# dfm/george

Measured on NVIDIA H100. Metric: gp.compute+log_likelihood N-points/sec, higher is better.
Workload: dtype f64

## Files before the change

george_b200/csrc/hodlr.cu:

```cuda
#include <algorithm>
#include <cmath>
#include <cstdlib>
#include <cstring>
#include <vector>

#include "common.cuh"
#include "hodlr_kernels.cuh"
#include "hodlr_lu.cuh"
#include "hodlr_aca2.cuh"
#include "hodlr_leaf.cuh"
#include "linalg.cuh"
#include "kernel_eval.cuh"

namespace bgp {
int upload_program(const DevProgram& P, DevBuf<DevProgram>& buf, cudaStream_t s);
int kmat_grad_contract_launch(const DevProgram* dprog, int nd, int np, const unsigned* which_dev, const double* x,
                              int64_t n, const double* M, int64_t ldm, const double* alpha, double ca, double cm,
                              double* g_dev, double* diag_dev, DevBuf<double>& scratch, cudaStream_t s);
int fill_identity_launch(double* A, int64_t n, cudaStream_t s);
int64_t grad_slab_partial_size(int64_t n, int64_t c, int np);
int64_t grad_slab_tile_size(int64_t n, int np);
int kmat_grad_slab_launch(const DevProgram* dprog, int nd, int np, const unsigned* which_dev, const double* x, int64_t n,
                          const double* W, int64_t j0, int64_t nc, int64_t jlo, int64_t jhi, const double* alpha,
                          double* partial, double* tile_part, double* diag_dev, cudaStream_t s);
// ... 10 lines not shown
                       const double* kdiag, double* var, DevBuf<double>& scratch, cudaStream_t s);
int kmat_x1_grad_matvec_launch(const DevProgram& P, const DevProgram* dprog, const double* x1, int64_t n1,
                               const double* x2, int64_t n2, const double* V, int64_t ldv, double scale, int add_prior,
                               double* out, DevBuf<double>& scratch, cudaStream_t s);
void predict_gemm_plan(int64_t m, int64_t nn, int64_t K, int64_t* nsplit_out, int64_t* klen_out);
int predict_gemm_sub(const double* A, int64_t lda, const double* B, int64_t ldb, int64_t m, int64_t nn, int64_t K,
                     bool lower, double* C, int64_t ldc, DevBuf<double>& slices, DevBuf<GemmDesc>& descs, cudaStream_t s);
bool comm_ready();
int comm_rank();
int comm_world();
int comm_allreduce_sum_f64(double* buf, size_t count, cudaStream_t s);
int comm_allgather_f64(const double* send, double* recv, size_t count, cudaStream_t s);
}
using namespace bgp;

struct HNode {
  int start, size, half, is_leaf, parent, dir, depth;
  int slot;
  int rank = 0, draws = 0, fallback = 0;
  int owned = 1;
  int top = 0;
};

struct PanelSet {
  DevBuf<double> V, U;
  int64_t ld = 0, row_off = 0;
  int vcols = 0, ucols = 0;
  double* vbase() const { return V.p - row_off; }
  double* ubase() const { return U.p - row_off; }
};

struct LevelInfo {
  std::vector<int> nodes;
  int set = 1;
  int cap = 0, max_cap = 0, vcol = 0, r = 0, ucol = 0;
  int max_half = 0, grow = 0;
  int desc_off = 0;
};

struct AcaGraphKey {
  A2Args a;
  int nn, ncc, nrc, shape, grid;
};

struct bgp_hodlr {
  cudaStream_t sA = nullptr, sB = nullptr;
  cudaEvent_t ev[8] = {nullptr};
  int64_t n = 0;
  int ndim = 0;
  bgp_hodlr_opts_t opts;
  bool computed = false;
  double log_det = 0.0;
  DevProgram prog;

  std::vector<HNode> nodes;
  std::vector<int> leaves;
  std::vector<LevelInfo> levels;
  std::vector<int> piv_off;
  std::vector<int> h_piv_rows, h_piv_cols;
  int max_leaf = 0, rtot = 0, vcols = 0, cut_depth = 0;
  int64_t row0 = 0, nloc = 0;
  std::vector<int64_t> shard_row0, shard_rows;
  bool top_pending = false;

  DevBuf<DevProgram> d_prog;
  DevBuf<double> d_x, d_yerr, d_diag, d_L, d_leaf_logdet, d_node_logdet, d_S, d_W, d_scalar, d_rhs;
  PanelSet top, loc;
  const PanelSet& pset(const LevelInfo& L) const { return L.set == 0 ? top : loc; }
  DevBuf<double> d_inv, d_gscratch;
  DevBuf<double> d_xsend, d_xrecv;
  DevBuf<unsigned> d_which;
  LuWorkspace lu_ws;
  DevBuf<GemmDesc> d_gram_desc, d_upd_desc;
  std::vector<NodeDesc> h_nodes;
  std::vector<int> cap_hint;
  int64_t cap_hint_n = -1;
  int cap_hint_min_size = -1;
  DevBuf<LeafDesc> d_leaves;
  DevBuf<AcaDesc> d_aca;
  DevBuf<AcaOut> d_aca_out;
  DevBuf<NodeDesc> d_nodes;
  DevBuf<PanelTile> d_ptiles;
  int small_limit = SS_MAX_N;
  bool leaf_cols_wide = false;
  DevBuf<int> d_idx, d_piv_rows, d_piv_cols, d_ticket, d_chain_done, d_ncols_by_depth;
  DevBuf<uint32_t> d_chain_state;
  DevBuf<A2Node> d_a2nodes;
  DevBuf<A2State> d_a2states;
  DevBuf<MT19937> d_a2rngs;
  DevBuf<A2EPart> d_epart;
  DevBuf<int> d_cand, d_cand_k, d_cand_words, d_cand_L, d_cand_next, d_cand_live, d_cchunk_node, d_rchunk_node, d_nactive;
  DevBuf<double> d_node_box;
  DevBuf<double2> d_cand_xu, d_gbox, d_cbox;
  DevBuf<unsigned long long> d_cmax, d_stats;
  DevBuf<int4> d_work;
  DevBuf<int> d_work_count, d_iter;
  AcaGraphKey aca_key;
  cudaGraph_t aca_graph = nullptr;
  cudaGraphExec_t aca_exec = nullptr;
  cudaStream_t sC = nullptr;
  bool profile = false;
  std::vector<cudaEvent_t> prof_events;
  double prof[12] = {0, 0, 0, 0, 0, 0, 0, 0, 0, 0, 0, 0};
  uint64_t draw_paths[4] = {0, 0, 0, 0};
  uint64_t eval_units[2] = {0, 0};
  DevBuf<double> d_vpart, d_upart, d_vmax;
  int aca_iters = 0;
  size_t w_cap = 0;

  double t_ms[5] = {0, 0, 0, 0, 0};
  double grad_t[4] = {0, 0, 0, 0};
  double work[6] = {0, 0, 0, 0, 0, 0};
};

static int ensure_streams(bgp_hodlr* h) {
  if (!h->sA) {
    BGP_CUDA(cudaStreamCreateWithFlags(&h->sA, cudaStreamNonBlocking));
    BGP_CUDA(cudaStreamCreateWithFlags(&h->sB, cudaStreamNonBlocking));
    for (int i = 0; i < 8; ++i) BGP_CUDA(cudaEventCreate(&h->ev[i]));
  }
  return BGP_OK;
}

static void build_tree(bgp_hodlr* h, int start, int size, int dir, int parent, int depth) {
  HNode nd;
  nd.start = start; nd.size = size; nd.half = size / 2; nd.dir = dir; nd.parent = parent; nd.depth = depth;
  nd.is_leaf = !(nd.half >= h->opts.min_size);
  nd.slot = 0;
  const int id = (int)h->nodes.size();
  h->nodes.push_back(nd);
  if (!nd.is_leaf) {
    build_tree(h, start, nd.half, 0, id, depth + 1);
    build_tree(h, start + nd.half, size - nd.half, 1, id, depth + 1);
  }
}

static int hodlr_solve_dev(bgp_hodlr* h, double* b, int64_t nrhs, int64_t ldb, cudaStream_t s, int part,
                           int64_t eye_row0 = -1);
static int hodlr_exchange_finish(bgp_hodlr* h);

static bool host_exchange(const bgp_hodlr* h) {
  return h->opts.shard_count > 1 &&
         !(comm_ready() && comm_world() == h->opts.shard_count && comm_rank() == h->opts.shard_rank);
}

static int reject_host_exchange(const bgp_hodlr* h, const char* what) {
  if (!host_exchange(h)) return BGP_OK;
  set_error("%s is not available on a host-exchange shard (shard %d of %d without a matching communicator): use "
            "bgp_hodlr_solve_local_dev / bgp_hodlr_solve_top_dev", what, h->opts.shard_rank, h->opts.shard_count);
  return BGP_ERR_INVALID;
}
static int hodlr_finish_top_impl(bgp_hodlr* h, bool allreduce);

constexpr size_t LS_SMEM_MAX = 200 * 1024;
constexpr int LS_MAX_LEAF = (int)(LS_SMEM_MAX / sizeof(double));

static bool leaf_solve_fits(int max_leaf, int cols) { return sizeof(double) * (size_t)max_leaf * cols <= LS_SMEM_MAX; }

static void set_sweep_func_attrs() {
  static std::atomic<uint64_t> done{0};
  int dev = 0;
  cudaGetDevice(&dev);
  const uint64_t bit = dev < 64 ? (1ull << dev) : 0;
  if (bit && (done.load(std::memory_order_relaxed) & bit)) return;
  cudaFuncSetAttribute(leaf_solve_kernel<1>, cudaFuncAttributeMaxDynamicSharedMemorySize, (int)LS_SMEM_MAX);
  cudaFuncSetAttribute(leaf_solve_kernel<2>, cudaFuncAttributeMaxDynamicSharedMemorySize, (int)LS_SMEM_MAX);
  cudaFuncSetAttribute(leaf_solve_kernel<4>, cudaFuncAttributeMaxDynamicSharedMemorySize, (int)LS_SMEM_MAX);
  cudaFuncSetAttribute(leaf_solve_kernel<LS_COLS>, cudaFuncAttributeMaxDynamicSharedMemorySize, (int)LS_SMEM_MAX);
  cudaFuncSetAttribute(leaf_solve_kernel<LS_COLS_WIDE>, cudaFuncAttributeMaxDynamicSharedMemorySize, (int)LS_SMEM_MAX);
  cudaFuncSetAttribute(small_solve_kernel, cudaFuncAttributeMaxDynamicSharedMemorySize, 160 * 1024);
  done.fetch_or(bit, std::memory_order_relaxed);
}

template <int COLS>
static int leaf_solve_launch(bgp_hodlr* h, double* X, int64_t ldx, const int* ncols_by_depth, int ncols_fixed,
                             int max_cols, cudaStream_t s, int l0, int l1) {
  const int ngroups = (max_cols + COLS - 1) / COLS;
  const dim3 grid((unsigned)((size_t)(l1 - l0) * (size_t)ngroups));
  const size_t smem = sizeof(double) * (size_t)h->max_leaf * COLS;
  leaf_solve_kernel<COLS><<<grid, LS_THREADS, smem, s>>>(h->d_leaves.p + l0, h->d_L.p, X, ldx, ncols_by_depth,
                                                         ncols_fixed, h->max_leaf, ngroups);
  BGP_LAUNCH_CHECK();
  return BGP_OK;
}

static int launch_leaf_solve(bgp_hodlr* h, double* X, int64_t ldx, const int* ncols_by_depth, int ncols_fixed,
                             int max_cols, cudaStream_t s, int l0 = 0, int l1 = -1) {
  if (l1 < 0) l1 = (int)h->leaves.size();
  const int nl = l1 - l0;
  if (nl <= 0 || max_cols == 0) return BGP_OK;
  const int m = h->max_leaf;
  if (h->leaf_cols_wide && max_cols > LS_COLS && leaf_solve_fits(m, LS_COLS_WIDE))
    return leaf_solve_launch<LS_COLS_WIDE>(h, X, ldx, ncols_by_depth, ncols_fixed, max_cols, s, l0, l1);
  int cols = max_cols <= 1 ? 1 : max_cols <= 2 ? 2 : max_cols <= 4 ? 4 : LS_COLS;
  while (cols > 1 && !leaf_solve_fits(m, cols)) cols /= 2;
  if (!leaf_solve_fits(m, cols)) {
    set_error("leaf size %d too large for the leaf solve kernel (at most %d rows)", m, LS_MAX_LEAF);
    return BGP_ERR_INVALID;
  }
  switch (cols) {
    case LS_COLS: return leaf_solve_launch<LS_COLS>(h, X, ldx, ncols_by_depth, ncols_fixed, max_cols, s, l0, l1);
    case 4: return leaf_solve_launch<4>(h, X, ldx, ncols_by_depth, ncols_fixed, max_cols, s, l0, l1);
    case 2: return leaf_solve_launch<2>(h, X, ldx, ncols_by_depth, ncols_fixed, max_cols, s, l0, l1);
    default: return leaf_solve_launch<1>(h, X, ldx, ncols_by_depth, ncols_fixed, max_cols, s, l0, l1);
  }
}

static int launch_level_big(bgp_hodlr* h, const LevelInfo& L, double* X, int64_t ldx, int ncolsW, int own_off, int factor,
                            int col_lo, int col_hi, cudaStream_t s, int b0, int b1);

static int launch_level(bgp_hodlr* h, const LevelInfo& L, double* X, int64_t ldx, int ncolsW, int own_off, int factor,
                        int col_lo, int col_hi, cudaStream_t s, int b0 = 0, int b1 = -1) {
  if (b1 < 0) b1 = (int)L.nodes.size();
  const int nn = b1 - b0;
  if (nn <= 0 || L.r == 0) {
    return BGP_OK;
  }
  const int r = L.r;
  const int64_t stride = (int64_t)2 * r * ncolsW;
  const size_t need = (size_t)nn * stride;
  if (need > h->w_cap) { set_error("internal: W workspace too small (%zu > %zu)", need, h->w_cap); return BGP_ERR_CUDA; }
  BGP_CUDA(cudaMemsetAsync(h->d_W.p, 0, sizeof(double) * need, s));
  if (2 * r > h->small_limit) return launch_level_big(h, L, X, ldx, ncolsW, own_off, factor, col_lo, col_hi, s, b0, b1);
  const NodeDesc* nd = h->d_nodes.p + L.desc_off + b0;
  const int max_nh = L.max_half + 1;
  if (r <= GTS_MAX_R) {
    dim3 grid((max_nh + GTS_ROWS - 1) / GTS_ROWS, nn * 2, (ncolsW + GTS_TC - 1) / GTS_TC);
    const double* vb = h->pset(L).vbase();
    const int64_t ldv = h->pset(L).ld;
    if (r <= 2) gram_tn_small_kernel<2><<<grid, GTS_THREADS, 0, s>>>(nd, vb, ldv, X, ldx, ncolsW, h->d_W.p, stride);
    else if (r <= 4) gram_tn_small_kernel<4><<<grid, GTS_THREADS, 0, s>>>(nd, vb, ldv, X, ldx, ncolsW, h->d_W.p, stride);
    else gram_tn_small_kernel<GTS_MAX_R><<<grid, GTS_THREADS, 0, s>>>(nd, vb, ldv, X, ldx, ncolsW, h->d_W.p, stride);
    BGP_LAUNCH_CHECK();
  } else {
    dim3 grid((max_nh + GT_CHUNK - 1) / GT_CHUNK, nn * 2, (ncolsW + GT_TC - 1) / GT_TC);
    gram_tn_kernel<<<grid, GT_THREADS, 0, s>>>(nd, h->pset(L).vbase(), h->pset(L).ld, X, ldx, ncolsW, h->d_W.p, stride);
    BGP_LAUNCH_CHECK();
  }
  {
    const size_t sbytes = sizeof(double) * (size_t)(2 * r) * (2 * r);
    small_solve_kernel<<<nn, SS_THREADS, sbytes, s>>>(nd, h->d_W.p, stride, ncolsW, own_off, factor, h->d_S.p,
                                                      h->d_node_logdet.p, L.desc_off + b0);
    BGP_LAUNCH_CHECK();
  }
  if (col_hi > col_lo) {
    dim3 grid((max_nh + UP_ROWS - 1) / UP_ROWS, nn * 2, (col_hi - col_lo + UP_TC - 1) / UP_TC);
    update_nn_kernel<<<grid, UP_THREADS, 0, s>>>(nd, h->pset(L).ubase(), h->pset(L).ld, X, ldx, col_lo, col_hi, h->d_W.p, stride, 0);
    BGP_LAUNCH_CHECK();
  }
  return BGP_OK;
}

static int launch_level_big(bgp_hodlr* h, const LevelInfo& L, double* X, int64_t ldx, int ncolsW, int own_off, int factor,
                            int col_lo, int col_hi, cudaStream_t s, int b0, int b1) {
  const int nn = b1 - b0;
  const int r = L.r, n2 = 2 * r;
  const int64_t stride = (int64_t)n2 * ncolsW;
  const int64_t ldv = h->pset(L).ld, ldu = h->pset(L).ld;
  double* W = h->d_W.p;
  constexpr int KCHUNK = 4096;
  std::vector<LuNode> lun(nn);
  std::vector<GemmDesc> gram, upd;
  int max_nh = 0;
  for (int k = 0; k < nn; ++k) {
    const int b = b0 + k;
    const HNode& nd = h->nodes[L.nodes[b]];
    const int64_t s_off = h->h_nodes[L.desc_off + b].s_off;
    lun[k].S = h->d_S.p + s_off;
    lun[k].piv = reinterpret_cast<int*>(lun[k].S + (int64_t)n2 * n2);
    lun[k].logdet = h->d_node_logdet.p + L.desc_off + b;
    double* Wn = W + (int64_t)k * stride;
    for (int hh = 0; hh < 2; ++hh) {
      const int rs = nd.start + (hh ? nd.half : 0), nh = hh ? (nd.size - nd.half) : nd.half;
      max_nh = std::max(max_nh, nh);
      for (int k0 = 0; k0 < nh; k0 += KCHUNK) {
        GemmDesc g;
// ... 202 lines not shown
    BGP_CUDA(cudaMemcpyAsync(act2, h->d_nactive.p, sizeof(int) * 2, cudaMemcpyDeviceToHost, s));
    BGP_CUDA(cudaStreamSynchronize(s));
    iters = it_host;
    g_launches.fetch_add((uint64_t)7 * (uint64_t)std::max(iters - 1, 0), std::memory_order_relaxed);
    if (act2[0] > 0) { set_error("ACA did not terminate"); return BGP_ERR_CUDA; }
  } else {
    while (active > 0) {
      for (int rep = 0; rep < 8; ++rep) {
        BGP_TRY(launch_iteration(s, 0, 0, h->profile ? iters : -1));
        iters++;
      }
      int act2[2] = {0, 0};
      BGP_CUDA(cudaMemcpyAsync(act2, h->d_nactive.p, sizeof(int) * 2, cudaMemcpyDeviceToHost, s));
      BGP_CUDA(cudaStreamSynchronize(s));
      active = act2[0];
      if (iters > (1 << 22)) { set_error("ACA did not terminate"); return BGP_ERR_CUDA; }
    }
  }
  h->aca_iters = iters;
  {
    unsigned long long st4[A2_NSTATS] = {0};
    BGP_CUDA(cudaMemcpyAsync(st4, h->d_stats.p, sizeof(st4), cudaMemcpyDeviceToHost, s));
    BGP_CUDA(cudaStreamSynchronize(s));
    for (int k = 0; k < 4; ++k) h->draw_paths[k] = st4[A2_PATH_REDO + k];
    h->eval_units[0] = st4[A2_UNITS_PULLED]; h->eval_units[1] = st4[A2_UNITS_LIVE];
    h->prof[1] = iters; h->prof[2] = (double)st4[0]; h->prof[3] = (double)st4[1]; h->prof[4] = (double)st4[2];
    h->prof[5] = (double)st4[3];
    if (h->profile) {
      double tot[6] = {0, 0, 0, 0, 0, 0};
      for (int i = 0; i < iters; ++i)
        for (int k = 0; k < 6; ++k) {
          float ms = 0;
          cudaEventElapsedTime(&ms, h->prof_events[(size_t)7 * i + k], h->prof_events[(size_t)7 * i + k + 1]);
          tot[k] += ms;
        }
      h->prof[0] = tot[0];
      for (int k = 0; k < 6; ++k) h->prof[6 + k] = tot[k];
    }
  }
  if (h->opts.exhaust_mode == BGP_EXHAUST_DENSE) {
    a2_dense_fill_kernel<<<dim3(nn, 64), 256, 0, s>>>(a);
    BGP_LAUNCH_CHECK();
    a2_dense_rank_kernel<<<(nn + 127) / 128, 128, 0, s>>>(a);
    BGP_LAUNCH_CHECK();
  }
  std::vector<A2State> hs(nn);
  BGP_CUDA(cudaMemcpyAsync(hs.data(), h->d_a2states.p, sizeof(A2State) * nn, cudaMemcpyDeviceToHost, s));
  BGP_CUDA(cudaStreamSynchronize(s));
  for (int i = 0; i < nn; ++i) {
    AcaOut o;
    o.rank = hs[i].rank; o.draws = hs[i].draws; o.fallback = hs[i].fallback; o.status = hs[i].status;
    houts[descs[i].node] = o;
  }
  return BGP_OK;
}

static int hodlr_compute_dev_impl(bgp_hodlr* h, const bgp_kernel_spec_t* spec, const double* x_dev, int64_t n,
                                  int32_t ndim, const double* yerr_dev, const bgp_hodlr_opts_t* opts_in) {
  h->computed = false;
  h->top_pending = false;
  for (uint64_t& c : h->draw_paths) c = 0;
  for (uint64_t& c : h->eval_units) c = 0;
  h->shard_row0.clear(); h->shard_rows.clear();
  BGP_TRY(require_device());
  BGP_TRY(ensure_streams(h));
  BGP_TRY(build_dev_program(spec, &h->prog));
  if (h->prog.ndim != ndim) { set_error("dimension mismatch: kernel ndim %d, input ndim %d", h->prog.ndim, ndim); return BGP_ERR_DIM; }
  if (ndim > ACA_MAX_NDIM) { set_error("HODLR supports at most %d input dimensions", ACA_MAX_NDIM); return BGP_ERR_INVALID; }
  if (n <= 0 || n > (int64_t)0x7fffffff) { set_error("invalid number of points %lld", (long long)n); return BGP_ERR_INVALID; }
  bgp_hodlr_opts_t o;
  if (opts_in) o = *opts_in; else bgp_hodlr_default_opts(&o);
  if (o.min_size < 1) { set_error("min_size must be >= 1"); return BGP_ERR_INVALID; }
  if (o.shard_count < 1) o.shard_count = 1;
  if (o.shard_count & (o.shard_count - 1)) { set_error("shard_count must be a power of two"); return BGP_ERR_INVALID; }
  if (o.shard_rank < 0 || o.shard_rank >= o.shard_count) { set_error("invalid shard_rank"); return BGP_ERR_INVALID; }
  if (o.shard_count > 1 && o.rng_mode == BGP_RNG_REFERENCE) { set_error("rng_mode=reference serialises the tree and cannot be sharded"); return BGP_ERR_INVALID; }
  h->opts = o;
  h->n = n;
  h->ndim = ndim;
  cudaStream_t sA = h->sA, sB = h->sB;
  set_sweep_func_attrs();
  h->small_limit = SS_MAX_N;
  if (const char* e = getenv("BGP_SMALL_RANK_LIMIT")) h->small_limit = std::min(SS_MAX_N, atoi(e));
  h->leaf_cols_wide = false;
  if (const char* e = getenv("BGP_LEAF_COLS")) h->leaf_cols_wide = atoi(e) > LS_COLS;

  h->nodes.clear(); h->leaves.clear(); h->levels.clear();
  h->nodes.reserve(2 * (size_t)(n / std::max(1, o.min_size)) + 8);
  build_tree(h, 0, (int)n, 0, -1, 0);
  int cut = 0;
  while ((1 << cut) < o.shard_count) cut++;
  h->cut_depth = cut;
  int max_depth = 0;
  for (auto& nd : h->nodes) max_depth = std::max(max_depth, nd.depth);
  h->row0 = 0; h->nloc = n;
  if (o.shard_count > 1) {
    int seen = 0; bool found = false;
    for (size_t i = 0; i < h->nodes.size(); ++i) {
      HNode& nd = h->nodes[i];
      if (nd.depth == cut) {
        if (seen == o.shard_rank) { h->row0 = nd.start; h->nloc = nd.size; found = true; }
        h->shard_row0.push_back(nd.start); h->shard_rows.push_back(nd.size);
        seen++;
      }
    }
    if (!found || seen != o.shard_count) {
      h->shard_row0.clear(); h->shard_rows.clear();
      set_error("tree too shallow to shard %d ways (N=%lld, min_size=%d)", o.shard_count, (long long)n, o.min_size);
      return BGP_ERR_INVALID;
    }
    for (auto& nd : h->nodes) {
      nd.top = nd.depth < cut;
      nd.owned = !nd.top && nd.start >= h->row0 && nd.start + nd.size <= h->row0 + h->nloc;
    }
  }
  h->levels.assign(max_depth + 1, LevelInfo());
  for (size_t i = 0; i < h->nodes.size(); ++i) {
    HNode& nd = h->nodes[i];
    if (nd.is_leaf) { if (nd.owned) { nd.slot = (int)h->leaves.size(); h->leaves.push_back((int)i); } continue; }
    if (!(nd.owned || nd.top)) continue;
    LevelInfo& L = h->levels[nd.depth];
    nd.slot = (int)L.nodes.size();
    L.nodes.push_back((int)i);
    L.max_half = std::max(L.max_half, nd.size - nd.half);
  }
  while (!h->levels.empty() && h->levels.back().nodes.empty()) h->levels.pop_back();
  const int nlev = (int)h->levels.size();
  for (int l = 0; l < nlev; ++l) h->levels[l].set = (o.shard_count > 1 && l < cut) ? 0 : 1;
  h->top.ld = n; h->top.row_off = 0;
  h->loc.ld = h->nloc; h->loc.row_off = h->row0;

  const int rcap0 = o.rank_capacity > 0 ? o.rank_capacity : 128;
  for (auto& L : h->levels) {
    int mh = 0;
    for (int id : L.nodes) mh = std::max(mh, h->nodes[id].half);
    L.max_cap = std::max(1, mh);
    L.cap = std::min(rcap0, L.max_cap);
  }
  if (o.rank_capacity <= 0 && h->cap_hint_n == n && h->cap_hint_min_size == o.min_size && (int)h->cap_hint.size() == nlev)
    for (int l = 0; l < nlev; ++l) h->levels[l].cap = std::min(h->levels[l].max_cap, std::max(h->levels[l].cap, h->cap_hint[l]));

  BGP_TRY(upload_program(h->prog, h->d_prog, sA));
  BGP_TRY(h->d_x.reserve((size_t)n * ndim, sA));
  BGP_TRY(h->d_diag.reserve((size_t)n, sA));
  if (x_dev != h->d_x.p) BGP_CUDA(cudaMemcpyAsync(h->d_x.p, x_dev, sizeof(double) * n * ndim, cudaMemcpyDeviceToDevice, sA));
  square_kernel<<<(unsigned)std::min<int64_t>((n + 255) / 256, 1184), 256, 0, sA>>>(yerr_dev, h->d_diag.p, n);
  BGP_LAUNCH_CHECK();
  BGP_CUDA(cudaEventRecord(h->ev[0], sA));

  const int nl = (int)h->leaves.size();
  std::vector<LeafDesc> hleaves(nl);
  int64_t loff = 0;
  h->max_leaf = 0;
  for (int i = 0; i < nl; ++i) {
    const HNode& nd = h->nodes[h->leaves[i]];
    hleaves[i].start = nd.start; hleaves[i].size = nd.size; hleaves[i].depth = nd.depth; hleaves[i]._pad = 0;
    hleaves[i].off = loff;
    loff += (int64_t)nd.size * nd.size;
    h->max_leaf = std::max(h->max_leaf, nd.size);
  }
  if (h->max_leaf > LS_MAX_LEAF) {
    set_error("leaf size %d too large: the leaf solve handles at most %d rows (N=%lld, min_size=%d); lower min_size",
              h->max_leaf, LS_MAX_LEAF, (long long)n, o.min_size);
    return BGP_ERR_INVALID;
  }
  BGP_TRY(h->d_leaves.reserve(std::max(nl, 1), sA));
  BGP_TRY(h->d_L.reserve((size_t)std::max<int64_t>(loff, 1), sA));
  BGP_TRY(h->d_leaf_logdet.reserve(std::max(nl, 1), sA));
  if (nl) {
    BGP_CUDA(cudaMemcpyAsync(h->d_leaves.p, hleaves.data(), sizeof(LeafDesc) * nl, cudaMemcpyHostToDevice, sA));
    const char* lf_env = getenv("BGP_LEAF_FACTOR");
    const bool generic = lf_env && strcmp(lf_env, "generic") == 0;
    if (h->max_leaf <= LF_MAX_LEAF && !generic) {
      leaf_factor_launch(h->prog.shape, nl, h->max_leaf, sA, h->d_prog.p, h->d_x.p, h->d_diag.p, h->d_leaves.p, h->d_L.p,
                         h->d_leaf_logdet.p);
    } else {
      leaf_build_factor_kernel<<<nl, LEAF_THREADS, 0, sA>>>(h->d_prog.p, h->d_x.p, h->d_diag.p, h->d_leaves.p, h->d_L.p,
                                                            h->d_leaf_logdet.p);
    }
    BGP_LAUNCH_CHECK();
  }
  BGP_CUDA(cudaEventRecord(h->ev[1], sA));

  std::vector<AcaDesc> hdesc;
  std::vector<int> desc_node;
  std::vector<AcaOut> houts;
  int64_t idx_total = 0, piv_total = 0;
  int nint = 0;
  BGP_CUDA(cudaStreamWaitEvent(sB, h->ev[1], 0));
  for (int attempt = 0;; ++attempt) {
    int vcols_set[2] = {0, 0};
    for (auto& L : h->levels) { L.vcol = vcols_set[L.set]; vcols_set[L.set] += L.cap; }
    h->top.vcols = vcols_set[0]; h->loc.vcols = vcols_set[1];
    h->vcols = vcols_set[0] + vcols_set[1];
    hdesc.clear(); desc_node.clear();
    h->piv_off.assign(h->nodes.size(), -1);
    idx_total = 0; piv_total = 0; nint = 0;
    for (int l = 0; l < nlev; ++l) {
      for (int id : h->levels[l].nodes) {
        const HNode& nd = h->nodes[id];
        AcaDesc d;
        d.row0 = nd.start + nd.half; d.n_rows = nd.size - nd.half; d.col0 = nd.start; d.n_cols = nd.half;
        d.vcol = h->levels[l].vcol; d.cap = h->levels[l].cap; d.pre_id = id; d.node = nint;
        d.idx_off = idx_total; d.piv_off = piv_total;
        h->piv_off[id] = (int)piv_total;
        idx_total += d.n_rows; piv_total += d.cap;
        hdesc.push_back(d); desc_node.push_back(id);
        nint++;
      }
    }
    std::vector<int> order(nint);
    for (int i = 0; i < nint; ++i) order[i] = i;
    if (o.rng_mode == BGP_RNG_REFERENCE) std::sort(order.begin(), order.end(), [&](int a, int b) { return hdesc[a].pre_id < hdesc[b].pre_id; });
    else std::stable_sort(order.begin(), order.end(), [&](int a, int b) {
      const int ta = h->nodes[hdesc[a].pre_id].top, tb = h->nodes[hdesc[b].pre_id].top;
      if (ta != tb) return ta > tb;
      return hdesc[a].n_rows > hdesc[b].n_rows;
    });
    std::vector<AcaDesc> hdesc_sorted(nint);
    for (int i = 0; i < nint; ++i) hdesc_sorted[i] = hdesc[order[i]];

    {
      const size_t need_top = (size_t)n * std::max(h->top.vcols, 1), need_loc = (size_t)h->nloc * std::max(h->loc.vcols, 1);
      if ((h->top.V.p && h->top.V.n < need_top) || (h->loc.V.p && h->loc.V.n < need_loc)) {
        if (h->top.V.n < need_top) h->top.V.release();
        if (h->loc.V.n < need_loc) h->loc.V.release();
        h->top.U.release(); h->loc.U.release();
        BGP_CUDA(cudaStreamSynchronize(sA)); BGP_CUDA(cudaStreamSynchronize(sB));
        cudaMemPool_t pool; int dev = 0;
        cudaGetDevice(&dev);
        if (cudaDeviceGetDefaultMemPool(&pool, dev) == cudaSuccess) cudaMemPoolTrimTo(pool, 0);
      }
      BGP_TRY(h->top.V.reserve(need_top, sB));
      BGP_TRY(h->loc.V.reserve(need_loc, sB));
    }
    BGP_TRY(h->d_aca.reserve(std::max(nint, 1), sB));
    BGP_TRY(h->d_aca_out.reserve(std::max(nint, 1), sB));
    BGP_TRY(h->d_idx.reserve((size_t)std::max<int64_t>(idx_total, 1), sB));
    BGP_TRY(h->d_piv_rows.reserve((size_t)std::max<int64_t>(piv_total, 1), sB));
    BGP_TRY(h->d_piv_cols.reserve((size_t)std::max<int64_t>(piv_total, 1), sB));
    BGP_TRY(h->d_ticket.reserve(1, sB));
    BGP_TRY(h->d_chain_state.reserve(640, sB));
    BGP_TRY(h->d_chain_done.reserve(std::max(nint, 1), sB));
    houts.assign(nint, AcaOut());
    if (nint && o.rng_mode != BGP_RNG_REFERENCE) {
      BGP_TRY(run_aca2(h, hdesc_sorted, houts, sB));
    } else if (nint) {
      BGP_CUDA(cudaMemcpyAsync(h->d_aca.p, hdesc_sorted.data(), sizeof(AcaDesc) * nint, cudaMemcpyHostToDevice, sB));
      BGP_CUDA(cudaMemsetAsync(h->d_ticket.p, 0, sizeof(int), sB));
      BGP_CUDA(cudaMemsetAsync(h->d_chain_done.p, 0, sizeof(int) * nint, sB));
      int maxcap = 1;
      for (auto& L : h->levels) maxcap = std::max(maxcap, L.cap);
      const size_t smem = ((sizeof(AcaShared) + 15) & ~size_t(15)) + sizeof(double) * (size_t)maxcap;
      cudaFuncSetAttribute(aca_kernel, cudaFuncAttributeMaxDynamicSharedMemorySize, 200 * 1024);
      if (smem > 200 * 1024) { set_error("rank capacity %d too large", maxcap); return BGP_ERR_RANK_CAPACITY; }
      aca_kernel<<<nint, ACA_THREADS, smem, sB>>>(h->d_prog.p, h->d_x.p, h->d_aca.p, nint, h->loc.vbase(), h->loc.ld, o.tol, (uint32_t)o.seed,
                                                  o.rng_mode, h->d_idx.p, h->d_piv_rows.p, h->d_piv_cols.p, h->d_aca_out.p,
                                                  h->d_ticket.p, h->d_chain_state.p, h->d_chain_done.p, o.exhaust_mode);
// ... 1048 lines not shown
```

george_b200/csrc/hodlr_kernels.cuh:

```cuda
#pragma once

#include <cooperative_groups.h>

#include "common.cuh"
#include "kernel_eval.cuh"

namespace bgp {

namespace cg = cooperative_groups;

struct MT19937 {
  uint32_t mt[624];
  int idx;
};
__device__ inline void mt_seed(MT19937& g, uint32_t s) {
  g.mt[0] = s;
  for (int i = 1; i < 624; ++i) g.mt[i] = 1812433253u * (g.mt[i - 1] ^ (g.mt[i - 1] >> 30)) + (uint32_t)i;
  g.idx = 624;
}
__device__ inline uint32_t mt_next(MT19937& g) {
  if (g.idx >= 624) {
    for (int i = 0; i < 624; ++i) {
      const uint32_t y = (g.mt[i] & 0x80000000u) | (g.mt[(i + 1) % 624] & 0x7fffffffu);
      g.mt[i] = g.mt[(i + 397) % 624] ^ (y >> 1) ^ ((y & 1u) ? 0x9908b0dfu : 0u);
// ... 71 lines not shown
      const double inv = 1.0 / d;
      __syncthreads();
      for (int i = k + 1 + threadIdx.x; i < nb; i += LEAF_THREADS) panel[i][k] *= inv;
      __syncthreads();
      for (int t = threadIdx.x; t < (nb - k - 1) * (nb - k - 1); t += LEAF_THREADS) {
        const int i = k + 1 + t % (nb - k - 1), j = k + 1 + t / (nb - k - 1);
        if (i >= j) panel[i][j] -= panel[i][k] * d * panel[j][k];
      }
      __syncthreads();
    }
    if (threadIdx.x < nb) {
      const double d = panel[threadIdx.x][threadIdx.x];
      dinv[threadIdx.x] = 1.0 / d;
      logdet += log(fabs(d));
    }
    for (int t = threadIdx.x; t < nb * nb; t += LEAF_THREADS) {
      const int i = t % nb, j = t / nb;
      if (i >= j) A[(int64_t)(k0 + j) * m + k0 + i] = panel[i][j];
    }
    __syncthreads();
    const int rem = m - k0 - nb;
    if (rem <= 0) break;
    for (int i = threadIdx.x; i < rem; i += LEAF_THREADS) {
      double* row = A + k0 + nb + i;
      double w[LEAF_NB];
#pragma unroll
      for (int j = 0; j < LEAF_NB; ++j) w[j] = (j < nb) ? row[(int64_t)(k0 + j) * m] : 0.0;
#pragma unroll
      for (int j = 0; j < LEAF_NB; ++j) {
        if (j < nb) {
          double s = w[j];
#pragma unroll
          for (int q = 0; q < j; ++q) s -= w[q] * panel[j][q];
          w[j] = s;
        }
      }
#pragma unroll
      for (int j = 0; j < LEAF_NB; ++j)
        if (j < nb) row[(int64_t)(k0 + j) * m] = w[j] * dinv[j];
    }
    __syncthreads();
    {
      const int tiles = (rem + 3) / 4;
      const double* Lp = A + (int64_t)k0 * m + k0 + nb;
      for (int t = threadIdx.x; t < tiles * tiles; t += LEAF_THREADS) {
        const int ti = t % tiles, tj = t / tiles;
        if (ti < tj) continue;
        double acc[4][4];
#pragma unroll
        for (int a = 0; a < 4; ++a)
#pragma unroll
          for (int b = 0; b < 4; ++b) acc[a][b] = 0.0;
        for (int q = 0; q < nb; ++q) {
          const double dq = panel[q][q];
          double li[4], lj[4];
#pragma unroll
          for (int a = 0; a < 4; ++a) {
            const int i = ti * 4 + a, j = tj * 4 + a;
            li[a] = (i < rem) ? Lp[(int64_t)q * m + i] : 0.0;
            lj[a] = (j < rem) ? Lp[(int64_t)q * m + j] * dq : 0.0;
          }
#pragma unroll
          for (int a = 0; a < 4; ++a)
#pragma unroll
            for (int b = 0; b < 4; ++b) acc[a][b] += li[a] * lj[b];
        }
#pragma unroll
        for (int b = 0; b < 4; ++b)
#pragma unroll
          for (int a = 0; a < 4; ++a) {
            const int i = ti * 4 + a, j = tj * 4 + b;
            if (i < rem && j < rem && i >= j) A[(int64_t)(k0 + nb + j) * m + k0 + nb + i] -= acc[a][b];
          }
      }
    }
    __syncthreads();
  }
  logdet = block_sum(logdet, red);
  if (threadIdx.x == 0) leaf_logdet[blockIdx.x] = logdet;
}

constexpr int LS_THREADS = 256;
constexpr int LS_COLS = 8;
constexpr int LS_COLS_WIDE = 32;
constexpr int LS_NB = 32;
constexpr int LS_BATCH = 4;

template <int COLS>
__global__ void __launch_bounds__(LS_THREADS, COLS <= LS_COLS ? 3 : 1) leaf_solve_kernel(const LeafDesc* __restrict__ leaves,
                                                                const double* __restrict__ Lbuf,
                                                                double* __restrict__ X, int64_t ldx,
                                                                const int* __restrict__ ncols_by_depth, int ncols_fixed,
                                                                int max_m, int ngroups) {
  extern __shared__ double xs[];
  __shared__ double sL[LS_NB][LS_NB + 1];
  const LeafDesc lf = leaves[blockIdx.x / ngroups];
  const int ncols = ncols_by_depth ? ncols_by_depth[lf.depth] : ncols_fixed;
  const int c0 = (blockIdx.x % ngroups) * COLS;
  if (c0 >= ncols) return;
  const int nc = min(COLS, ncols - c0);
  const int m = lf.size;
  const double* A = Lbuf + lf.off;
  const int lane = threadIdx.x & 31, warp = threadIdx.x >> 5;
  constexpr int NW = LS_THREADS / 32;
  for (int t = threadIdx.x; t < m * COLS; t += LS_THREADS) {
    const int i = t % m, c = t / m;
    xs[c * max_m + i] = (c < nc) ? X[(int64_t)(c0 + c) * ldx + lf.start + i] : 0.0;
  }
  for (int kb = 0; kb < m; kb += LS_NB) {
    const int nb = min(LS_NB, m - kb);
    __syncthreads();
    for (int t = threadIdx.x; t < LS_NB * LS_NB; t += LS_THREADS) {
      const int i = t % LS_NB, k = t / LS_NB;
      sL[i][k] = (i < nb && k < nb && i > k) ? A[(int64_t)(kb + k) * m + kb + i] : 0.0;
    }
    __syncthreads();
    for (int c = warp; c < nc; c += NW) {
      double y = (lane < nb) ? xs[c * max_m + kb + lane] : 0.0;
      for (int k = 0; k < nb; ++k) {
        const double yk = __shfl_sync(0xffffffffu, y, k);
        if (lane > k) y -= sL[lane][k] * yk;
      }
      if (lane < nb) xs[c * max_m + kb + lane] = y;
    }
    __syncthreads();
    const int r0 = kb + nb;
    for (int i = r0 + threadIdx.x; i < m; i += LS_THREADS) {
      double acc[COLS];
#pragma unroll
      for (int c = 0; c < COLS; ++c) acc[c] = 0.0;
      const double* Li = A + (int64_t)kb * m + i;
#pragma unroll 8
      for (int k = 0; k < nb; ++k) {
        const double l = Li[(int64_t)k * m];
#pragma unroll
        for (int c = 0; c < COLS; ++c) acc[c] += l * xs[c * max_m + kb + k];
      }
#pragma unroll
      for (int c = 0; c < COLS; ++c) if (c < nc) xs[c * max_m + i] -= acc[c];
    }
  }
  __syncthreads();
  for (int t = threadIdx.x; t < m * nc; t += LS_THREADS) {
    const int i = t % m, c = t / m;
    xs[c * max_m + i] /= A[(int64_t)i * m + i];
  }
  const int nblk = (m + LS_NB - 1) / LS_NB;
  for (int b = nblk - 1; b >= 0; --b) {
    const int kb = b * LS_NB;
    const int nb = min(LS_NB, m - kb);
    const int r0 = kb + nb;
    __syncthreads();
    for (int t = threadIdx.x; t < LS_NB * LS_NB; t += LS_THREADS) {
      const int i = t % LS_NB, k = t / LS_NB;
      sL[i][k] = (i < nb && k < nb && i > k) ? A[(int64_t)(kb + k) * m + kb + i] : 0.0;
    }
    for (int k = warp; k < nb; k += NW) {
      double acc[COLS];
#pragma unroll
      for (int c = 0; c < COLS; ++c) acc[c] = 0.0;
      const double* Lk = A + (int64_t)(kb + k) * m;
      for (int i0 = r0 + lane; i0 < m; i0 += 32 * LS_BATCH) {
        double l[LS_BATCH];
#pragma unroll
        for (int j = 0; j < LS_BATCH; ++j) l[j] = (i0 + 32 * j < m) ? Lk[i0 + 32 * j] : 0.0;
#pragma unroll
        for (int j = 0; j < LS_BATCH; ++j) {
          const int i = i0 + 32 * j;
          if (i < m) {
#pragma unroll
            for (int c = 0; c < COLS; ++c) acc[c] += l[j] * xs[c * max_m + i];
          }
// ... 646 lines not shown
```

george_b200/csrc/hodlr_leaf.cuh:

```cuda
#pragma once

#include "gemm_dmma.cuh"
#include "hodlr_kernels.cuh"

namespace bgp {

constexpr int LF_THREADS = 256;
constexpr int LF_NB = 32;
constexpr int LF_MAX_LEAF = 768;

__host__ __device__ inline int lf_panel_ld(int max_m) { return ((max_m + 15) / 16) * 16 + 4; }

template <int SHAPE>
__global__ void __launch_bounds__(LF_THREADS, 2) leaf_factor_kernel(const DevProgram* __restrict__ gprog,
                                                                    const double* __restrict__ x,
                                                                    const double* __restrict__ diag,
                                                                    const LeafDesc* __restrict__ leaves,
                                                                    double* __restrict__ Lbuf,
                                                                    double* __restrict__ leaf_logdet, int ldp) {
  extern __shared__ __align__(16) double lf_smem[];
  double* pn = lf_smem;
  double* dall = lf_smem + LF_NB * ldp;
  DevProgram* P = reinterpret_cast<DevProgram*>(lf_smem + (LF_NB + 1) * ldp);
  __shared__ double red[32];
// ... 57 lines not shown
          for (int b = 0; b < 4; ++b)
#pragma unroll
            for (int e = 0; e < 2; ++e) {
              const int c = b * 8 + 2 * lc + e;
              if (i < rem && c < nb && i >= c) pn[c * ldp + i] -= acc[a][b][e];
            }
        }
      }
      __syncthreads();
    }
    if (warp == 0) {
      double w[LF_NB];
#pragma unroll
      for (int j = 0; j < LF_NB; ++j) w[j] = (j <= lane && lane < nb) ? pn[j * ldp + lane] : 0.0;
#pragma unroll
      for (int k = 0; k < LF_NB; ++k) {
        if (k < nb) {
          const double d = __shfl_sync(0xffffffffu, w[k], k);
          const double l = (lane > k && lane < nb) ? w[k] / d : 0.0;
          if (lane > k) w[k] = l;
          const double ld = l * d;
#pragma unroll
          for (int j = k + 1; j < LF_NB; ++j) {
            const double lj = __shfl_sync(0xffffffffu, l, j);
            if (j <= lane) w[j] -= ld * lj;
          }
        }
      }
      if (lane < nb) {
        double* col = A + (int64_t)k0 * m + k0 + lane;
        double d = 0.0;
#pragma unroll
        for (int j = 0; j < LF_NB; ++j) {
          if (j < lane) { pn[j * ldp + lane] = w[j]; col[(int64_t)j * m] = w[j]; }
          if (j == lane) d = w[j];
        }
        col[(int64_t)lane * m] = d;
        dall[k0 + lane] = d;
        dinv[lane] = 1.0 / d;
        logdet += log(fabs(d));
      }
    }
    __syncthreads();
    const volatile double* l11 = pn;
    for (int i = LF_NB + threadIdx.x; i < rem; i += LF_THREADS) {
      double w[LF_NB];
#pragma unroll
      for (int j = 0; j < LF_NB; ++j) w[j] = pn[j * ldp + i];
#pragma unroll
      for (int j = 0; j < LF_NB; ++j) {
        double s = w[j];
#pragma unroll
        for (int q = 0; q < j; ++q) s -= w[q] * l11[q * ldp + j];
        w[j] = s;
      }
      double* row = A + (int64_t)k0 * m + k0 + i;
#pragma unroll
      for (int j = 0; j < LF_NB; ++j) row[(int64_t)j * m] = w[j] * dinv[j];
    }
    __syncthreads();
  }
  logdet = block_sum(logdet, red);
  if (threadIdx.x == 0) leaf_logdet[blockIdx.x] = logdet;
}

__host__ inline size_t lf_smem_bytes(int shape, int max_m) {
  return sizeof(double) * (size_t)(LF_NB + 1) * lf_panel_ld(max_m) + (shape == BGP_SHAPE_GENERIC ? sizeof(DevProgram) : 0);
}

template <int SHAPE>
inline void leaf_factor_launch_shape(int n_leaves, int max_m, cudaStream_t s, const DevProgram* prog, const double* x,
                                     const double* diag, const LeafDesc* leaves, double* L, double* leaf_logdet) {
  const size_t smem = lf_smem_bytes(SHAPE, max_m);
  cudaFuncSetAttribute(leaf_factor_kernel<SHAPE>, cudaFuncAttributeMaxDynamicSharedMemorySize, (int)smem);
  leaf_factor_kernel<SHAPE><<<n_leaves, LF_THREADS, smem, s>>>(prog, x, diag, leaves, L, leaf_logdet, lf_panel_ld(max_m));
}

inline void leaf_factor_launch(int shape, int n_leaves, int max_m, cudaStream_t s, const DevProgram* prog,
                               const double* x, const double* diag, const LeafDesc* leaves, double* L,
                               double* leaf_logdet) {
  BGP_SHAPE_SWITCH(shape, (leaf_factor_launch_shape<SHAPE>(n_leaves, max_m, s, prog, x, diag, leaves, L, leaf_logdet)));
}

}
```

Before: 22.73 million.

## Invert leaf LDL factors explicitly and apply them with tensor-core GEMMs

After the blocked leaf LDL factorization, a new kernel overwrites each leaf's unit lower factor with its explicit inverse, using per-warp triangular inverses of the diagonal blocks and DMMA products for the off-diagonal blocks. Leaf solves then run as two dense triangular matrix products with a diagonal scaling in between (leaf_apply_kernel), replacing the sequential substitution kernel. The intent is to turn latency-bound triangular solves into tensor-core GEMMs. The cost is an extra inverse pass at factor time, possible loss of numerical accuracy from explicit inversion, and removal of the optional wide-column solve path.

```diff
diff --git a/george_b200/csrc/hodlr.cu b/george_b200/csrc/hodlr.cu
--- a/george_b200/csrc/hodlr.cu
+++ b/george_b200/csrc/hodlr.cu
@@ -116,7 +116,7 @@
   DevBuf<NodeDesc> d_nodes;
   DevBuf<PanelTile> d_ptiles;
   int small_limit = SS_MAX_N;
-  bool leaf_cols_wide = false;
+  bool leaf_inv = false;
   DevBuf<int> d_idx, d_piv_rows, d_piv_cols, d_ticket, d_chain_done, d_ncols_by_depth;
   DevBuf<uint32_t> d_chain_state;
   DevBuf<A2Node> d_a2nodes;
@@ -201,7 +201,9 @@
   cudaFuncSetAttribute(leaf_solve_kernel<2>, cudaFuncAttributeMaxDynamicSharedMemorySize, (int)LS_SMEM_MAX);
   cudaFuncSetAttribute(leaf_solve_kernel<4>, cudaFuncAttributeMaxDynamicSharedMemorySize, (int)LS_SMEM_MAX);
   cudaFuncSetAttribute(leaf_solve_kernel<LS_COLS>, cudaFuncAttributeMaxDynamicSharedMemorySize, (int)LS_SMEM_MAX);
-  cudaFuncSetAttribute(leaf_solve_kernel<LS_COLS_WIDE>, cudaFuncAttributeMaxDynamicSharedMemorySize, (int)LS_SMEM_MAX);
+  cudaFuncSetAttribute(leaf_apply_kernel<1>, cudaFuncAttributeMaxDynamicSharedMemorySize, (int)LS_SMEM_MAX);
+  cudaFuncSetAttribute(leaf_apply_kernel<2>, cudaFuncAttributeMaxDynamicSharedMemorySize, (int)LS_SMEM_MAX);
+  cudaFuncSetAttribute(leaf_apply_kernel<4>, cudaFuncAttributeMaxDynamicSharedMemorySize, (int)LS_SMEM_MAX);
   cudaFuncSetAttribute(small_solve_kernel, cudaFuncAttributeMaxDynamicSharedMemorySize, 160 * 1024);
   done.fetch_or(bit, std::memory_order_relaxed);
 }
@@ -218,14 +220,28 @@
   return BGP_OK;
 }
 
+template <int NB8>
+static int leaf_apply_launch(bgp_hodlr* h, double* X, int64_t ldx, const int* ncols_by_depth, int ncols_fixed,
+                             int max_cols, cudaStream_t s, int l0, int l1) {
+  const int ngroups = (max_cols + 8 * NB8 - 1) / (8 * NB8);
+  const dim3 grid((unsigned)((size_t)(l1 - l0) * (size_t)ngroups));
+  leaf_apply_kernel<NB8><<<grid, LA_THREADS, la_smem_bytes(h->max_leaf, 8 * NB8), s>>>(
+      h->d_leaves.p + l0, h->d_L.p, X, ldx, ncols_by_depth, ncols_fixed, la_ld(h->max_leaf), ngroups);
+  BGP_LAUNCH_CHECK();
+  return BGP_OK;
+}
+
 static int launch_leaf_solve(bgp_hodlr* h, double* X, int64_t ldx, const int* ncols_by_depth, int ncols_fixed,
                              int max_cols, cudaStream_t s, int l0 = 0, int l1 = -1) {
   if (l1 < 0) l1 = (int)h->leaves.size();
   const int nl = l1 - l0;
   if (nl <= 0 || max_cols == 0) return BGP_OK;
+  if (h->leaf_inv) {
+    if (max_cols <= 8) return leaf_apply_launch<1>(h, X, ldx, ncols_by_depth, ncols_fixed, max_cols, s, l0, l1);
+    if (max_cols <= 16) return leaf_apply_launch<2>(h, X, ldx, ncols_by_depth, ncols_fixed, max_cols, s, l0, l1);
+    return leaf_apply_launch<4>(h, X, ldx, ncols_by_depth, ncols_fixed, max_cols, s, l0, l1);
+  }
   const int m = h->max_leaf;
-  if (h->leaf_cols_wide && max_cols > LS_COLS && leaf_solve_fits(m, LS_COLS_WIDE))
-    return leaf_solve_launch<LS_COLS_WIDE>(h, X, ldx, ncols_by_depth, ncols_fixed, max_cols, s, l0, l1);
   int cols = max_cols <= 1 ? 1 : max_cols <= 2 ? 2 : max_cols <= 4 ? 4 : LS_COLS;
   while (cols > 1 && !leaf_solve_fits(m, cols)) cols /= 2;
   if (!leaf_solve_fits(m, cols)) {
@@ -594,8 +610,7 @@
   set_sweep_func_attrs();
   h->small_limit = SS_MAX_N;
   if (const char* e = getenv("BGP_SMALL_RANK_LIMIT")) h->small_limit = std::min(SS_MAX_N, atoi(e));
-  h->leaf_cols_wide = false;
-  if (const char* e = getenv("BGP_LEAF_COLS")) h->leaf_cols_wide = atoi(e) > LS_COLS;
+  h->leaf_inv = false;
 
   h->nodes.clear(); h->leaves.clear(); h->levels.clear();
   h->nodes.reserve(2 * (size_t)(n / std::max(1, o.min_size)) + 8);
@@ -683,9 +698,12 @@
     BGP_CUDA(cudaMemcpyAsync(h->d_leaves.p, hleaves.data(), sizeof(LeafDesc) * nl, cudaMemcpyHostToDevice, sA));
     const char* lf_env = getenv("BGP_LEAF_FACTOR");
     const bool generic = lf_env && strcmp(lf_env, "generic") == 0;
-    if (h->max_leaf <= LF_MAX_LEAF && !generic) {
+    h->leaf_inv = h->max_leaf <= LF_MAX_LEAF && !generic;
+    if (h->leaf_inv) {
       leaf_factor_launch(h->prog.shape, nl, h->max_leaf, sA, h->d_prog.p, h->d_x.p, h->d_diag.p, h->d_leaves.p, h->d_L.p,
                          h->d_leaf_logdet.p);
+      BGP_LAUNCH_CHECK();
+      leaf_inverse_launch(nl, sA, h->d_leaves.p, h->d_L.p);
     } else {
       leaf_build_factor_kernel<<<nl, LEAF_THREADS, 0, sA>>>(h->d_prog.p, h->d_x.p, h->d_diag.p, h->d_leaves.p, h->d_L.p,
                                                             h->d_leaf_logdet.p);
diff --git a/george_b200/csrc/hodlr_kernels.cuh b/george_b200/csrc/hodlr_kernels.cuh
--- a/george_b200/csrc/hodlr_kernels.cuh
+++ b/george_b200/csrc/hodlr_kernels.cuh
@@ -177,12 +177,11 @@
 
 constexpr int LS_THREADS = 256;
 constexpr int LS_COLS = 8;
-constexpr int LS_COLS_WIDE = 32;
 constexpr int LS_NB = 32;
 constexpr int LS_BATCH = 4;
 
 template <int COLS>
-__global__ void __launch_bounds__(LS_THREADS, COLS <= LS_COLS ? 3 : 1) leaf_solve_kernel(const LeafDesc* __restrict__ leaves,
+__global__ void __launch_bounds__(LS_THREADS, 3) leaf_solve_kernel(const LeafDesc* __restrict__ leaves,
                                                                 const double* __restrict__ Lbuf,
                                                                 double* __restrict__ X, int64_t ldx,
                                                                 const int* __restrict__ ncols_by_depth, int ncols_fixed,
diff --git a/george_b200/csrc/hodlr_leaf.cuh b/george_b200/csrc/hodlr_leaf.cuh
--- a/george_b200/csrc/hodlr_leaf.cuh
+++ b/george_b200/csrc/hodlr_leaf.cuh
@@ -163,4 +163,230 @@
   BGP_SHAPE_SWITCH(shape, (leaf_factor_launch_shape<SHAPE>(n_leaves, max_m, s, prog, x, diag, leaves, L, leaf_logdet)));
 }
 
-}
+constexpr int LI_THREADS = 256;
+constexpr int LI_WARPS = LI_THREADS / 32;
+constexpr int LI_DLD = LF_NB + 1;
+constexpr int LI_TLD = LF_NB + 4;
+constexpr size_t LI_SMEM_BYTES = sizeof(double) * LI_WARPS * LF_NB * LI_DLD;
+
+__device__ __forceinline__ double linv_at(const double* A, int m, int i, int j) {
+  return i > j ? A[(int64_t)i * m + j] : (i == j ? 1.0 : 0.0);
+}
+
+__global__ void __launch_bounds__(LI_THREADS) leaf_inverse_kernel(const LeafDesc* __restrict__ leaves,
+                                                                  double* __restrict__ Lbuf) {
+  extern __shared__ __align__(16) double li_smem[];
+  const LeafDesc lf = leaves[blockIdx.x];
+  const int m = lf.size;
+  double* A = Lbuf + lf.off;
+  const int lane = threadIdx.x & 31, warp = threadIdx.x >> 5;
+  const int nblk = (m + LF_NB - 1) / LF_NB;
+
+  double* sl = li_smem + warp * LF_NB * LI_DLD;
+  for (int J = warp; J < nblk; J += LI_WARPS) {
+    const int k0 = J * LF_NB, nb = min(LF_NB, m - k0);
+    for (int t = lane; t < LF_NB * LF_NB; t += 32) {
+      const int i = t % LF_NB, q = t / LF_NB;
+      sl[i * LI_DLD + q] = (i < nb && q < i) ? A[(int64_t)(k0 + q) * m + k0 + i] : 0.0;
+    }
+    __syncwarp();
+    double x[LF_NB];
+#pragma unroll
+    for (int i = 0; i < LF_NB; ++i) {
+      double s = (i == lane) ? 1.0 : 0.0;
+#pragma unroll
+      for (int q = 0; q < i; ++q) s -= sl[i * LI_DLD + q] * x[q];
+      x[i] = s;
+    }
+#pragma unroll
+    for (int i = 0; i < LF_NB; ++i)
+      if (i > lane && i < nb) A[(int64_t)(k0 + i) * m + k0 + lane] = x[i];
+    __syncwarp();
+  }
+
+  double* st = li_smem + warp * 16 * LI_TLD;
+  const int lr = lane >> 2, lc = lane & 3;
+  for (int J = nblk - 2; J >= 0; --J) {
+    __syncthreads();
+    const int c0 = J * LF_NB, R0 = c0 + LF_NB;
+    const int ntl = (m - R0 + 15) / 16;
+    for (int t = warp; t < ntl; t += LI_WARPS) {
+      const int r0 = R0 + 16 * t, kend = min(r0 + 16, m);
+      double acc[2][4][2];
+#pragma unroll
+      for (int a = 0; a < 2; ++a)
+#pragma unroll
+        for (int b = 0; b < 4; ++b) { acc[a][b][0] = 0.0; acc[a][b][1] = 0.0; }
+#pragma unroll 4
+      for (int k0 = R0; k0 < kend; k0 += 4) {
+        const int k = k0 + lc;
+        double af[2], bf[4];
+#pragma unroll
+        for (int a = 0; a < 2; ++a) {
+          const int row = r0 + a * 8 + lr;
+          af[a] = (row < m && k <= row) ? linv_at(A, m, row, k) : 0.0;
+        }
+#pragma unroll
+        for (int b = 0; b < 4; ++b) bf[b] = k < m ? A[(int64_t)(c0 + b * 8 + lr) * m + k] : 0.0;
+#pragma unroll
+        for (int a = 0; a < 2; ++a)
+#pragma unroll
+          for (int b = 0; b < 4; ++b) dmma884(acc[a][b][0], acc[a][b][1], af[a], bf[b]);
+      }
+#pragma unroll
+      for (int a = 0; a < 2; ++a)
+#pragma unroll
+        for (int b = 0; b < 4; ++b)
+#pragma unroll
+          for (int e = 0; e < 2; ++e) st[(a * 8 + lr) * LI_TLD + b * 8 + 2 * lc + e] = acc[a][b][e];
+      __syncwarp();
+#pragma unroll
+      for (int a = 0; a < 2; ++a)
+#pragma unroll
+        for (int b = 0; b < 4; ++b) { acc[a][b][0] = 0.0; acc[a][b][1] = 0.0; }
+#pragma unroll
+      for (int q0 = 0; q0 < LF_NB; q0 += 4) {
+        const int q = q0 + lc;
+        double af[2], bf[4];
+#pragma unroll
+        for (int a = 0; a < 2; ++a) af[a] = st[(a * 8 + lr) * LI_TLD + q];
+#pragma unroll
+        for (int b = 0; b < 4; ++b) bf[b] = linv_at(A, m, c0 + q, c0 + b * 8 + lr);
+#pragma unroll
+        for (int a = 0; a < 2; ++a)
+#pragma unroll
+          for (int b = 0; b < 4; ++b) dmma884(acc[a][b][0], acc[a][b][1], af[a], bf[b]);
+      }
+#pragma unroll
+      for (int a = 0; a < 2; ++a) {
+        const int row = r0 + a * 8 + lr;
+        if (row < m)
+#pragma unroll
+          for (int b = 0; b < 4; ++b)
+#pragma unroll
+            for (int e = 0; e < 2; ++e) A[(int64_t)row * m + c0 + b * 8 + 2 * lc + e] = -acc[a][b][e];
+      }
+      __syncwarp();
+    }
+  }
+}
+
+inline void leaf_inverse_launch(int n_leaves, cudaStream_t s, const LeafDesc* leaves, double* L) {
+  cudaFuncSetAttribute(leaf_inverse_kernel, cudaFuncAttributeMaxDynamicSharedMemorySize, (int)LI_SMEM_BYTES);
+  leaf_inverse_kernel<<<n_leaves, LI_THREADS, LI_SMEM_BYTES, s>>>(leaves, L);
+}
+
+constexpr int LA_THREADS = 512;
+constexpr int LA_WARPS = LA_THREADS / 32;
+
+template <int NB8>
+__global__ void __launch_bounds__(LA_THREADS, 2) leaf_apply_kernel(const LeafDesc* __restrict__ leaves,
+                                                                const double* __restrict__ Lbuf,
+                                                                double* __restrict__ X, int64_t ldx,
+                                                                const int* __restrict__ ncols_by_depth,
+                                                                int ncols_fixed, int ld, int ngroups) {
+  constexpr int COLS = 8 * NB8;
+  extern __shared__ __align__(16) double la_xs[];
+  const LeafDesc lf = leaves[blockIdx.x / ngroups];
+  const int ncols = ncols_by_depth ? ncols_by_depth[lf.depth] : ncols_fixed;
+  const int cg = (blockIdx.x % ngroups) * COLS;
+  if (cg >= ncols) return;
+  const int nc = min(COLS, ncols - cg);
+  const int m = lf.size;
+  const double* A = Lbuf + lf.off;
+  double* Xl = X + (int64_t)cg * ldx + lf.start;
+  const int lane = threadIdx.x & 31, warp = threadIdx.x >> 5;
+  const int lr = lane >> 2, lc = lane & 3;
+  for (int t = threadIdx.x; t < m * COLS; t += LA_THREADS) {
+    const int i = t % m, c = t / m;
+    la_xs[c * ld + i] = (c < nc) ? Xl[(int64_t)c * ldx + i] : 0.0;
+  }
+  __syncthreads();
+  const int ntiles = (m + 15) / 16;
+  double acc[2][NB8][2];
+
+  for (int base = ntiles - 1; base >= 0; base -= LA_WARPS) {
+    const int t = base - warp;
+#pragma unroll
+    for (int a = 0; a < 2; ++a)
+#pragma unroll
+      for (int b = 0; b < NB8; ++b) { acc[a][b][0] = 0.0; acc[a][b][1] = 0.0; }
+    if (t >= 0) {
+      const int r0 = 16 * t, kend = min(r0 + 16, m);
+#pragma unroll 4
+      for (int k0 = 0; k0 < kend; k0 += 4) {
+        const int k = k0 + lc;
+        double af[2], bf[NB8];
+#pragma unroll
+        for (int a = 0; a < 2; ++a) {
+          const int row = r0 + a * 8 + lr;
+          af[a] = (row < m && k <= row) ? linv_at(A, m, row, k) : 0.0;
+        }
+#pragma unroll
+        for (int b = 0; b < NB8; ++b) bf[b] = k < m ? la_xs[(b * 8 + lr) * ld + k] : 0.0;
+#pragma unroll
+        for (int a = 0; a < 2; ++a)
+#pragma unroll
+          for (int b = 0; b < NB8; ++b) dmma884(acc[a][b][0], acc[a][b][1], af[a], bf[b]);
+      }
+    }
+    __syncthreads();
+    if (t >= 0) {
+#pragma unroll
+      for (int a = 0; a < 2; ++a) {
+        const int row = 16 * t + a * 8 + lr;
+        if (row < m) {
+          const double d = A[(int64_t)row * m + row];
+#pragma unroll
+          for (int b = 0; b < NB8; ++b)
+#pragma unroll
+            for (int e = 0; e < 2; ++e) la_xs[(b * 8 + 2 * lc + e) * ld + row] = acc[a][b][e] / d;
+        }
+      }
+    }
+    __syncthreads();
+  }
+
+  for (int base = 0; base < ntiles; base += LA_WARPS) {
+    const int t = base + warp;
+    if (t >= ntiles) break;
+    const int r0 = 16 * t;
+#pragma unroll
+    for (int a = 0; a < 2; ++a)
+#pragma unroll
+      for (int b = 0; b < NB8; ++b) { acc[a][b][0] = 0.0; acc[a][b][1] = 0.0; }
+#pragma unroll 4
+    for (int k0 = r0; k0 < m; k0 += 4) {
+      const int k = k0 + lc;
+      double af[2], bf[NB8];
+#pragma unroll
+      for (int a = 0; a < 2; ++a) {
+        const int row = r0 + a * 8 + lr;
+        af[a] = (k < m && k >= row) ? linv_at(A, m, k, row) : 0.0;
+      }
+#pragma unroll
+      for (int b = 0; b < NB8; ++b) bf[b] = k < m ? la_xs[(b * 8 + lr) * ld + k] : 0.0;
+#pragma unroll
+      for (int a = 0; a < 2; ++a)
+#pragma unroll
+        for (int b = 0; b < NB8; ++b) dmma884(acc[a][b][0], acc[a][b][1], af[a], bf[b]);
+    }
+#pragma unroll
+    for (int a = 0; a < 2; ++a) {
+      const int row = r0 + a * 8 + lr;
+      if (row < m)
+#pragma unroll
+        for (int b = 0; b < NB8; ++b)
+#pragma unroll
+          for (int e = 0; e < 2; ++e) {
+            const int c = b * 8 + 2 * lc + e;
+            if (c < nc) Xl[(int64_t)c * ldx + row] = acc[a][b][e];
+          }
+    }
+  }
+}
+
+__host__ __device__ inline int la_ld(int max_m) { return lf_panel_ld(max_m); }
+__host__ inline size_t la_smem_bytes(int max_m, int cols) { return sizeof(double) * (size_t)la_ld(max_m) * cols; }
+
+}
```

Measured after the change: 23.37 million, median of 6. +2.8%, better.
